# jkelleyrtp/ofdm

Hardware: AMD Instinct MI355X
Metric: complex IQ Msamples/s through RX demod (higher is better)
Workload: dtype f32; 1 GPU; cfg2: 64-subcarrier 64QAM guard-band frames, RX demod only (CP strip+FFT64+pilot phase+demap); frames_per_gpu=1000000, symbols_per_frame=16, samples_per_frame=1280, parallelism=frame-index split x1, no collective

## Files before the change

ofdm_amd/csrc/kernels_n64.hip:

```cpp
#include "device_common.hpp"
#include "kernels.hpp"
#include <type_traits>
#include <mutex>
#include <stdlib.h>

namespace ofdm {

typedef float f32x2 __attribute__((ext_vector_type(2)));
typedef __attribute__((address_space(3))) f32x2 *lds_cf_ptr;
typedef __attribute__((address_space(3))) unsigned *lds_u32_ptr;
template <int BPS, bool GUARD, bool HK, int BURST = 1>
__global__ __launch_bounds__(256, 4) void k_demod64(Fast64Params p) {
    constexpr int S = 80, CP = 16;
    constexpr int ND = GUARD ? 48 : 64;
    constexpr int REGION_DW = ND * BPS / 4;
    constexpr int SLAB = 8 * 72;

    __shared__ cf slab_all[4 * SLAB];
    __shared__ __align__(16) unsigned img_all[4 * BURST * REGION_DW];

    const int lane = threadIdx.x & 63;
    const int wave = __builtin_amdgcn_readfirstlane(threadIdx.x >> 6);
    const int s = lane >> 3, t = lane & 7;
    cf *buf = slab_all + wave * SLAB + s * 72;
    unsigned *img0 = img_all + wave * BURST * REGION_DW;

    cf w[7];
#pragma unroll
    for (int r = 1; r < 8; ++r) w[r - 1] = p.tw[r * t];
    cf g[8];
    if (HK) {
#pragma unroll
        for (int m = 0; m < 8; ++m) {
            cf h = p.hk[t + 8 * m];
            float ns = h.x * h.x + h.y * h.y;
            g[m] = make_float2(h.x / ns, -h.y / ns);
        }
    }
    unsigned wa[8], ra[8], fa[8], fs[8];
#pragma unroll
    for (int r = 0; r < 8; ++r) {
        wa[r] = pinned(lds_addr(buf + (swz(8 * t) ^ r)));
        ra[r] = pinned(lds_addr(buf + 8 * r + (t ^ r)));
        const int c = t + 8 * r;
        const int q = GUARD ? data_classes_below64(c) : c;
        const int bo = (s * ND + q) * BPS;
        const bool data = carrier_class64(c, GUARD) == 0;
        fa[r] = pinned(lds_addr(img0 + (bo >> 5)));
        fs[r] = pinned(data ? (unsigned)(bo & 31) : 0xFFFFFFFFu);
    }
    const int lane_off = s * S + t;

    auto group = [&](long long f, int kk, unsigned img_off) {
        const cf *src = p.in + f * p.frame_stride + (long long)(p.first_symbol + kk * 8) * S + CP + lane_off;
        cf v[8];
#pragma unroll
        for (int m = 0; m < 8; ++m) v[m] = src[8 * m];
        bfly8<false>(v);
        if (kProfile && p.debug == 3) {
            float acc = 0.f;
#pragma unroll
            for (int m = 0; m < 8; ++m) acc += v[m].x + v[m].y;
            if (acc == 12345.678f) p.out[0] = 1;
            return;
        }
#pragma unroll
        for (int r = 0; r < 8; ++r) *(lds_cf_ptr)(unsigned long)wa[r] = f32x2{v[r].x, v[r].y};
#pragma unroll
        for (int m = 0; m < 8; ++m) { const f32x2 q = *(lds_cf_ptr)(unsigned long)ra[m]; v[m] = make_float2(q.x, q.y); }
#pragma unroll
        for (int r = 1; r < 8; ++r) v[r] = cmul(v[r], w[r - 1]);
        bfly8<false>(v);
        if (HK) {
#pragma unroll
            for (int m = 0; m < 8; ++m) v[m] = cmul(v[m], g[m]);
        }
        cf rot = make_float2(1.f, 0.f);
        if (GUARD) {
            cf pv = make_float2(1.f, 0.f);
            pv = (t == 6) ? v[0] : pv;
            pv = (t == 1) ? v[3] : pv;
            pv = (t == 7) ? v[4] : pv;
            pv = (t == 2) ? v[7] : pv;
            const float turns = sum8_lanes(__ocml_atan2pi_f32(pv.y, pv.x)) * 0.125f;
            rot = make_float2(__builtin_amdgcn_cosf(turns), -__builtin_amdgcn_sinf(turns));
        }
        if (kProfile && p.debug == 2) {
            float acc = 0.f;
#pragma unroll
            for (int m = 0; m < 8; ++m) acc += v[m].x + v[m].y;
            if (acc == 12345.678f) p.out[0] = 1;
            return;
        }
        unsigned *img = reinterpret_cast<unsigned *>(reinterpret_cast<unsigned char *>(img0) + img_off);
        for (int i = lane; i < REGION_DW; i += 64) img[i] = 0u;
#pragma unroll
        for (int m = 0; m < 8; ++m) {
            const bool all_data = !GUARD || m == 1 || m == 2 || m == 5 || m == 6;
            if (all_data || fs[m] != 0xFFFFFFFFu) {
                const unsigned idx = GUARD ? demap_point_rot(v[m], rot, BPS) : demap_point(v[m], BPS);
                const lds_u32_ptr wd = (lds_u32_ptr)(unsigned long)(fa[m] + img_off);
                __hip_atomic_fetch_or(wd, idx << fs[m], __ATOMIC_RELAXED, __HIP_MEMORY_SCOPE_WORKGROUP);
                if (BPS > 1 && (32 % BPS) != 0) {
                    if (fs[m] + BPS > 32) __hip_atomic_fetch_or(wd + 1, idx >> (32 - fs[m]), __ATOMIC_RELAXED, __HIP_MEMORY_SCOPE_WORKGROUP);
                }
            }
        }
    };
    auto store_image = [&](unsigned *dst, int ndw) {
        if (kProfile && (p.debug == 1 || p.debug == 2 || p.debug == 3)) { if (img0[lane] == 0x12345678u) dst[0] = 1u; return; }
        if (kProfile && p.debug == 4) dst = reinterpret_cast<unsigned *>(p.out) + (blockIdx.x & 255) * 4 * BURST * REGION_DW + wave * BURST * REGION_DW;
        if (kProfile && p.debug == 5) { for (int i = lane; i < ndw; i += 64) __builtin_nontemporal_store(img0[i], dst + i); return; }
        if ((REGION_DW % 4) == 0 && p.wide_stores) {
            if (p.store_policy) {
                typedef unsigned v4u __attribute__((ext_vector_type(4)));
                for (int i = lane; i < ndw / 4; i += 64) {
                    const v4u val = reinterpret_cast<const v4u *>(img0)[i];
                    uint4 *a = reinterpret_cast<uint4 *>(dst) + i;
                    if (p.store_policy == 1) asm volatile("global_store_dwordx4 %0, %1, off nt" ::"v"(a), "v"(val) : "memory");
                    else if (p.store_policy == 2) asm volatile("global_store_dwordx4 %0, %1, off sc1" ::"v"(a), "v"(val) : "memory");
                    else asm volatile("global_store_dwordx4 %0, %1, off sc0 sc1" ::"v"(a), "v"(val) : "memory");
                }
                return;
            }
            for (int i = lane; i < ndw / 4; i += 64) reinterpret_cast<uint4 *>(dst)[i] = reinterpret_cast<const uint4 *>(img0)[i];
        } else for (int i = lane; i < ndw; i += 64) dst[i] = img0[i];
    };

    if (BURST > 1) {
        const long long n_bursts = p.n_groups / BURST;
        for (long long j = (long long)blockIdx.x * 4 + wave; j < n_bursts; j += p.stride_groups) {
            const long long g0 = j * BURST;
            long long f = g0 / p.groups_per_frame;
            int kk = (int)(g0 - f * p.groups_per_frame);
#pragma nounroll
            for (int b = 0; b < BURST; ++b) {
                group(f, kk, (unsigned)(b * REGION_DW * 4));
                if (++kk == p.groups_per_frame) { kk = 0; ++f; }
            }
            store_image(reinterpret_cast<unsigned *>(p.out + g0 * (long long)(REGION_DW * 4)), BURST * REGION_DW);
        }
        return;
    }

    long long f = p.f0 + (long long)blockIdx.x * p.blk_df + wave * p.wave_df;
    int kk = p.k0 + (int)((blockIdx.x * (long long)p.blk_dk + wave * p.wave_dk));
    f += kk / p.groups_per_frame;
    kk %= p.groups_per_frame;
    for (long long g_idx = (long long)blockIdx.x * 4 + wave; g_idx < p.n_groups; g_idx += p.stride_groups) {
        group(f, kk, 0u);
        store_image(reinterpret_cast<unsigned *>(p.out + f * p.out_stride + (long long)kk * 8 * (ND * BPS / 8)), REGION_DW);
        f += p.step_df;
        kk += p.step_dk;
        if (kk >= p.groups_per_frame) { kk -= p.groups_per_frame; f += 1; }
    }
}

struct RxFrame64Params {
    const float2 *in;
    long long n_frames, frame_stride, frame_len;
    const int32_t *offset;
    const double *f_delta;
    const int32_t *nsym;
    const float2 *tw, *inv_training;
    unsigned char *out;
    long long out_stride;
    float2 *hk;
    unsigned char *final_out;
    long long final_stride;
    int32_t *final_len;
    const int32_t *frame_list;
    const int32_t *frame_count;
    int32_t *cut_list;
    int32_t *cut_count;
};

__device__ __forceinline__ cf lane_xor_sum(cf v) {
    v.x += dpp_f<0x128>(v.x); v.y += dpp_f<0x128>(v.y);
    v.x += __shfl_xor(v.x, 16, 64); v.y += __shfl_xor(v.y, 16, 64);
    v.x += __shfl_xor(v.x, 32, 64); v.y += __shfl_xor(v.y, 32, 64);
    return v;
}

template <int BPS, bool GUARD, int MODE>
__global__ __launch_bounds__(256, (MODE == 0 && GUARD) ? 4 : 3) void k_rxframe64(RxFrame64Params p) {
    constexpr int S = 80, CP = 16;
    constexpr int ND = GUARD ? 48 : 64;
    constexpr int SYM_BYTES = ND * BPS / 8;
    constexpr int REGION_DW = ND * BPS / 4;
    constexpr int SLAB = 8 * 72;
    __shared__ cf slab_all[4 * SLAB];
    __shared__ cf ginv_all[4 * 64];
    __shared__ unsigned img_all[4 * REGION_DW];

    const int lane = threadIdx.x & 63;
    const int wave = __builtin_amdgcn_readfirstlane(threadIdx.x >> 6);
    const int s = lane >> 3, t = lane & 7;
    cf *buf = slab_all + wave * SLAB + s * 72;
    unsigned *img = img_all + wave * REGION_DW;

    __shared__ cf twl[64];
    __shared__ int bofftab[8 * 64];
    if (threadIdx.x < 64) twl[threadIdx.x] = p.tw[threadIdx.x];
    if (wave == 0) {
#pragma unroll
        for (int m = 0; m < 8; ++m) {
            const int c = t + 8 * m;
            const int q = GUARD ? data_classes_below64(c) : c;
            bofftab[m * 64 + lane] = (carrier_class64(c, GUARD) == 0) ? (s * ND + q) * BPS : -1;
        }
    }
    __shared__ int cutbuf[4][1 + 16];
    if (MODE == 0 && lane == 0) cutbuf[wave][0] = 0;
    __syncthreads();
    const int wr = swz(8 * t);
    auto cut_flush = [&]() {
        const int m = cutbuf[wave][0];
        if (m > 0) {
            const int base = atomicAdd(p.cut_count, m);
            for (int i = 0; i < m; ++i) p.cut_list[base + i] = cutbuf[wave][1 + i];
            cutbuf[wave][0] = 0;
        }
    };

    const long long n_items = p.frame_list ? (long long)*p.frame_count : p.n_frames;
    const long long istep = (long long)gridDim.x * 4;
    const int vzero = pinned(0);
    long long f_n = 0; int ns_v = 0, off_v = 0; double fd_v = 0.0;
    auto fetch_scalars = [&](long long item) {
        if (item < n_items) {
            f_n = p.frame_list ? (long long)p.frame_list[item] : item;
            const long long fi = f_n + vzero;
            ns_v = p.nsym[fi];
            off_v = p.offset ? p.offset[fi] : 0;
            fd_v = p.f_delta ? p.f_delta[fi] : 0.0;
        }
    };
    fetch_scalars((long long)blockIdx.x * 4 + wave);
    for (long long item = (long long)blockIdx.x * 4 + wave; item < n_items; item += istep) {
        const long long f = f_n;
        const int ns = __builtin_amdgcn_readfirstlane(ns_v);
        const long long off = __builtin_amdgcn_readfirstlane(off_v);
        const double turns = __hiloint2double(__builtin_amdgcn_readfirstlane(__double2hiint(fd_v)), __builtin_amdgcn_readfirstlane(__double2loint(fd_v))) * 0.15915494309189533577;
        fetch_scalars(item + istep);
        if (ns <= 0) { if (p.final_out && lane == 0) p.final_len[f] = 0; continue; }
        const cf st = cfo_phasor(turns, 8);
        int keep = 0;
        const cf *src = p.in + f * p.frame_stride + off;
        const long long avail = p.frame_len - off;

        auto frame_body = [&](auto cut_tag) {
        constexpr bool CUT = decltype(cut_tag)::value;
        const cf *safe = p.in + f * p.frame_stride + t;
        auto issue_group = [&](int k0, cf *v, unsigned &zmask) {
            const int count = ns - k0 < 8 ? ns - k0 : 8;
            const int n0 = (10 + k0 + s) * S + CP + t;
            const cf *base = s < count ? src + n0 : safe;
            zmask = 0u;
#pragma unroll
            for (int m = 0; m < 8; ++m) {
                const bool pad = CUT && s < count && (n0 + 8 * m) >= avail;
                v[m] = ld_cf(pad ? safe : base + 8 * m);
                if (CUT) zmask |= pad ? 1u << m : 0u;
            }
        };
        cf *ginv = ginv_all + wave * 64;
        cf v[8];
        unsigned zm = 0u;
        {
            cf tws[6];
            const int lq = pinned(lane);
#pragma unroll
            for (int q = 0; q < 6; ++q) {
                const int h = 32 >> q;
                const cf x = twl[(lq & (h - 1)) << q];
                tws[q] = (lane & h) ? x : make_float2(1.f, 0.f);
            }
            const int bin = bitrev6(lane);
            const cf invt = p.inv_training[bin];
            const int nb = 5 * S + CP + lane;
            cf xb[5];
#pragma unroll
            for (int b = 0; b < 5; ++b) xb[b] = ld_cf((!CUT || (nb + S * b) < avail) ? src + nb + S * b : safe);
            issue_group(0, v, zm);
#pragma unroll
            for (int b = 0; b < 5; ++b) if (CUT && (nb + S * b) >= avail) xb[b] = make_float2(0.f, 0.f);
            cf acc;
            if (p.f_delta) {
                const cf s80 = cfo_phasor(turns, S), q0 = cfo_phasor(turns, nb);
                acc = cadd(cmul(xb[4], s80), xb[3]);
                acc = cadd(cmul(acc, s80), xb[2]);
                acc = cadd(cmul(acc, s80), xb[1]);
                acc = cadd(cmul(acc, s80), xb[0]);
                acc = cmul(acc, q0);
            } else acc = cadd(cadd(cadd(xb[4], xb[3]), cadd(xb[2], xb[1])), xb[0]);
            acc = lane_fft64(acc, lane, tws);
            cf h = cmul(acc, invt);
            h = make_float2(h.x * 0.2f, h.y * 0.2f);
            if (p.hk) p.hk[f * 64 + bin] = h;
            const float rn = __builtin_amdgcn_rcpf(h.x * h.x + h.y * h.y);
            wave_fence();
            ginv[bin] = make_float2(h.x * rn, -h.y * rn);
            wave_fence();
        }
        for (int k0 = 0; k0 < ns; k0 += 8) {
            const int count = ns - k0 < 8 ? ns - k0 : 8;
            const int n0 = (10 + k0 + s) * S + CP + t;
            cf vn[8];
            unsigned zn = 0u;
            issue_group(k0 + 8 < ns ? k0 + 8 : k0, vn, zn);
            if (CUT && zm) {
#pragma unroll
                for (int m = 0; m < 8; ++m) if ((zm >> m) & 1u) v[m] = make_float2(0.f, 0.f);
            }
            if (p.f_delta) {
                cf ph = cfo_phasor(turns, n0);
#pragma unroll
                for (int m = 0; m < 8; ++m) { v[m] = cmul(v[m], ph); ph = cmul(ph, st); }
            }
            bfly8<false>(v);
#pragma unroll
            for (int r = 0; r < 8; ++r) buf[wr ^ r] = v[r];
#pragma unroll
            for (int m = 0; m < 8; ++m) v[m] = buf[8 * m + (t ^ m)];
#pragma unroll
            for (int r = 1; r < 8; ++r) v[r] = cmul(v[r], twl[r * t]);
            bfly8<false>(v);
#pragma unroll
            for (int m = 0; m < 8; ++m) v[m] = cmul(v[m], ginv[t + 8 * m]);
            cf rot = make_float2(1.f, 0.f);
            if (GUARD) {
                cf pv = make_float2(1.f, 0.f);
                pv = (t == 6) ? v[0] : pv;
                pv = (t == 1) ? v[3] : pv;
                pv = (t == 7) ? v[4] : pv;
                pv = (t == 2) ? v[7] : pv;
                const float trn = sum8_lanes(__ocml_atan2pi_f32(pv.y, pv.x)) * 0.125f;
                rot = make_float2(__builtin_amdgcn_cosf(trn), -__builtin_amdgcn_sinf(trn));
            }
            for (int i = lane; i < REGION_DW; i += 64) img[i] = 0u;
#pragma unroll
            for (int m = 0; m < 8; ++m) {
                const int bo = bofftab[m * 64 + lane];
                if (bo >= 0) {
                    const unsigned idx = GUARD ? demap_point_rot(v[m], rot, BPS) : demap_point(v[m], BPS);
                    or_field<BPS>(img, bo, idx);
                }
            }
#pragma unroll
            for (int m = 0; m < 8; ++m) v[m] = vn[m];
            zm = zn;
            const int ndw = (count * SYM_BYTES + 3) / 4;
            if (p.final_out) {
                wave_fence();
                if (k0 == 0) {
                    const unsigned long long lo = (unsigned long long)img[0] | ((unsigned long long)img[1] << 32);
                    const unsigned long long hi = (unsigned long long)img[2] | ((unsigned long long)img[3] << 32);
                    const int body = ns * SYM_BYTES - 16;
                    keep = OFDM_HEADER_KEEP(int, lo, hi, body);
                    if (lane == 0) p.final_len[f] = keep;
                }
                unsigned char *fo = p.final_out + f * p.final_stride;
                for (int i = lane; i < ndw; i += 64) {
                    const int ob = k0 * SYM_BYTES + 4 * i - 16;
                    if (ob < 0 || ob >= keep) continue;
                    if (ob + 4 <= keep) *reinterpret_cast<unsigned *>(fo + ob) = img[i];
                    else for (int j = 0; ob + j < keep; ++j) fo[ob + j] = (unsigned char)(img[i] >> (8 * j));
                }
            } else {
                unsigned *dst = reinterpret_cast<unsigned *>(p.out + f * p.out_stride + (long long)k0 * SYM_BYTES);
                for (int i = lane; i < ndw; i += 64) dst[i] = img[i];
            }
        }
        };
        const bool whole = (long long)(10 + ns) * S <= avail;
        if (MODE == 0) {
            if (whole) frame_body(std::false_type{});
            else if (lane == 0) {
                const int m = cutbuf[wave][0];
                cutbuf[wave][1 + m] = (int32_t)f;
                cutbuf[wave][0] = m + 1;
                if (m + 1 == 16) cut_flush();
            }
        } else if (MODE == 1) {
            if (!whole) frame_body(std::true_type{});
        } else {
            if (whole) frame_body(std::false_type{}); else frame_body(std::true_type{});
        }
    }
    if (MODE == 0 && lane == 0) cut_flush();
}

template <int BPS, bool GUARD> static hipError_t launch_rxframe(RxFrame64Params p, dim3 grid, hipStream_t st, bool split) {
    if (!split) { hipLaunchKernelGGL((k_rxframe64<BPS, GUARD, 2>), grid, dim3(256), 0, st, p); return hipGetLastError(); }
    hipError_t e = hipMemsetAsync(p.cut_count, 0, sizeof(int32_t), st);
    if (e != hipSuccess) return e;
    hipLaunchKernelGGL((k_rxframe64<BPS, GUARD, 0>), grid, dim3(256), 0, st, p);
    if ((e = hipGetLastError()) != hipSuccess) return e;
    p.frame_list = p.cut_list; p.frame_count = p.cut_count;
    hipLaunchKernelGGL((k_rxframe64<BPS, GUARD, 1>), grid, dim3(256), 0, st, p);
    return hipGetLastError();
}

hipError_t run_rxframe64(const SymParams &sp, float2 *hk_out, hipStream_t st, int num_cu, unsigned char *final_out,
                         long long final_stride, int32_t *final_len, const int32_t *frame_list, const int32_t *frame_count,
                         int32_t *cut_ws) {
    const int nd = sp.guard ? 48 : 64;
    if ((nd * sp.bps) % 16 != 0 || !sp.nsym_frame || sp.soft) return hipErrorNotSupported;
    const bool to_final = final_out && final_len && (reinterpret_cast<uintptr_t>(final_out) & 3) == 0 && (final_stride & 3) == 0;
    if (!to_final && ((reinterpret_cast<uintptr_t>(sp.out_bytes) & 3) || (sp.out_stride & 3))) return hipErrorNotSupported;
    if (sp.n_frames <= 0) return hipSuccess;
    RxFrame64Params p;
    p.in = sp.in; p.n_frames = sp.n_frames; p.frame_stride = sp.frame_stride; p.frame_len = sp.frame_len;
    p.offset = sp.offset; p.f_delta = sp.f_delta; p.nsym = sp.nsym_frame; p.tw = sp.tw; p.inv_training = sp.inv_training;
    p.out = sp.out_bytes; p.out_stride = sp.out_stride; p.hk = hk_out;
    p.final_out = nullptr; p.final_stride = 0; p.final_len = nullptr;
    if (to_final) { p.final_out = final_out; p.final_stride = final_stride; p.final_len = final_len; }
    else if (final_out) return hipErrorNotSupported;
    p.frame_list = frame_list; p.frame_count = frame_count;
    const bool roomy = sp.frame_len >= (long long)(10 + sp.syms_per_frame) * 80 + 64;
    const bool split = cut_ws != nullptr && frame_list == nullptr && roomy && !tuning_or_default(sp.tune).no_rxframe64_split;
    p.cut_count = split ? cut_ws : nullptr; p.cut_list = split ? cut_ws + 4 : nullptr;
    const dim3 grid((unsigned)persistent_grid((sp.n_frames + 3) / 4, frame_list ? 64 : (long long)num_cu * 8, tuning_or_default(sp.tune)));
    trace_add(sp.trace, frame_list ? "k_rxframe64<list>" : (p.final_out ? "k_rxframe64<finish>" : "k_rxframe64"));
    if (split) trace_add(sp.trace, "k_rxframe64<cut,list>");
    return with_bps(sp.bps, [&](auto B) { return with_bool(sp.guard != 0, [&](auto G) {
        return launch_rxframe<decltype(B)::value, decltype(G)::value>(p, grid, st, split); }); });
}

struct TxFrame64Params {
    const uint8_t *payload;
    long long payload_stride;
    const int32_t *payload_len;
    int payload_bytes;
    long long n_frames;
    int n_sym;
    const float2 *tw;
    const float2 *header;
    float header_max;
    float2 *out;
    long long out_stride;
    int debug;
};

template <int BPS, bool GUARD>
__global__ __launch_bounds__(256, 4) void k_txframe64(TxFrame64Params p) {
    constexpr int S = 80, CP = 16, HDR = 10 * S;
    constexpr int ND = GUARD ? 48 : 64;
    constexpr int SYM_BITS = ND * BPS;
    extern __shared__ __align__(16) unsigned char smem[];
    cf *hd = reinterpret_cast<cf *>(smem);
    cf *fb = hd + HDR;
    const int groups = (p.n_sym + 7) >> 3;
    unsigned *mxw = reinterpret_cast<unsigned *>(fb + (size_t)groups * 8 * S);
    unsigned *sbw_all = mxw + 4;
    const int sbw_dw = groups * 128 + 8;
    const int stream_dw = groups * 8 * (SYM_BITS / 8) / 4 + 1;

    const int tid = threadIdx.x, lane = tid & 63, nthr = blockDim.x, nwaves = nthr >> 6;
    const int wave = __builtin_amdgcn_readfirstlane(tid >> 6);
    const int s = lane >> 3, t = lane & 7;
    cf w[7];
#pragma unroll
    for (int r = 1; r < 8; ++r) { const cf x = p.tw[r * t]; w[r - 1] = make_float2(x.x, -x.y); }
    int qoff[8];
#pragma unroll
    for (int m = 0; m < 8; ++m) {
        const int c = t + 8 * m, cls = carrier_class64(c, GUARD);
        qoff[m] = cls == 0 ? (GUARD ? data_classes_below64(c) : c) * BPS : (cls == 2 ? -2 : -1);
    }
    const int wr = swz(8 * t);
    for (int i = tid; i < HDR; i += nthr) hd[i] = p.header[i];
    __shared__ float lvl[16];
    if (tid < 16) lvl[tid] = BPS > 1 && tid < (1 << (BPS >> 1)) ? axis_level((unsigned)tid, BPS >> 1) : 0.f;

    const bool aligned = ((reinterpret_cast<uintptr_t>(p.payload) | (uintptr_t)p.payload_stride) & 3) == 0;
    auto pay_dword = [&](const uint8_t *pay, long long len, int i) -> unsigned {
        const long long b0 = 4LL * i;
        if (b0 + 4 <= len && aligned) return reinterpret_cast<const unsigned *>(pay)[i];
        unsigned v = 0;
        for (int j = 0; j < 4; ++j) if (b0 + j < len) v |= (unsigned)pay[b0 + j] << (8 * j);
        return v;
    };
    const int vzero = pinned(0);
    const bool row0 = aligned && 4LL * tid + 4 <= p.payload_bytes, row1 = aligned && 4LL * (tid + nthr) + 4 <= p.payload_bytes;
    auto issue = [&](long long fr, unsigned &d0, unsigned &d1, int &ln) {
        const long long fc = fr < p.n_frames ? fr : p.n_frames - 1;
        const uint8_t *row = p.payload + fc * p.payload_stride;
        d0 = *reinterpret_cast<const unsigned *>(row0 ? row + 4 * tid : reinterpret_cast<const uint8_t *>(p.tw));
        d1 = *reinterpret_cast<const unsigned *>(row1 ? row + 4 * (tid + nthr) : reinterpret_cast<const uint8_t *>(p.tw));
        ln = p.payload_len ? p.payload_len[fc + vzero] : p.payload_bytes;
    };
    auto settle = [&](unsigned raw, bool whole, const uint8_t *pay, long long len, int i) -> unsigned {
        const long long keep = len - 4LL * i;
        if (whole) return keep >= 4 ? raw : (keep <= 0 ? 0u : raw & ((1u << (8 * (int)keep)) - 1u));
        return pay_dword(pay, len, i);
    };
    auto fill = [&](unsigned *sbw, long long fr, unsigned d0, unsigned d1, long long len) {
        const uint8_t *pay = p.payload + fr * p.payload_stride;
        if (tid < 4) sbw[tid] = tid < 2 ? (unsigned)((unsigned long long)len >> (32 * tid)) : 0u;
        if (tid + 4 < stream_dw) sbw[4 + tid] = settle(d0, row0, pay, len, tid);
        if (tid + nthr + 4 < stream_dw) sbw[4 + tid + nthr] = settle(d1, row1, pay, len, tid + nthr);
        for (int i = tid + 2 * nthr; i + 4 < stream_dw; i += nthr) sbw[4 + i] = pay_dword(pay, len, i);
    };
    long long f = blockIdx.x;
    unsigned pre0 = 0, pre1 = 0;
    int pre_len = 0;
    long long len = 0;
    int cur = 0;
    if (f < p.n_frames) {
        issue(f, pre0, pre1, pre_len);
        len = row_len(__builtin_amdgcn_readfirstlane(pre_len), p.payload_bytes);
        fill(sbw_all, f, pre0, pre1, len);
        issue(f + gridDim.x, pre0, pre1, pre_len);
    }
    if (tid < 2) mxw[tid] = 0u;
    for (; f < p.n_frames; f += gridDim.x, cur ^= 1) {
        lds_barrier();
        const long long t0 = kProfile && p.debug ? (long long)__builtin_amdgcn_s_memtime() : 0;
        const unsigned char *sb = reinterpret_cast<const unsigned char *>(sbw_all + cur * sbw_dw);
        long long t1 = 0;
        const int npoints = (int)(((16 + len) * 8 + BPS - 1) / BPS);
        float lmax = 0.f;
        for (int g = wave; g < groups; g += nwaves) {
            const int k = 8 * g + s;
            cf *buf = fb + k * S;
            cf v[8];
#pragma unroll
            for (int m = 0; m < 8; ++m) {
                cf z = make_float2(0.f, 0.f);
                if (qoff[m] == -2) z = make_float2(1.f, 0.f);
                else if (qoff[m] >= 0) {
                    const int bit = k * SYM_BITS + qoff[m];
                    if (bit < npoints * BPS && k < p.n_sym) {
                        const unsigned two = (unsigned)sb[bit >> 3] | ((unsigned)sb[(bit >> 3) + 1] << 8);
                        const unsigned idx = (two >> (bit & 7)) & ((1u << BPS) - 1u);
                        z = BPS == 1 ? map_point(idx, 1) : make_float2(lvl[idx & ((1u << (BPS >> 1)) - 1u)], lvl[idx >> (BPS >> 1)]);
                    }
                }
                v[m] = z;
            }
            bfly8<true>(v);
#pragma unroll
            for (int r = 0; r < 8; ++r) buf[wr ^ r] = v[r];
#pragma unroll
            for (int m = 0; m < 8; ++m) v[m] = buf[8 * m + (t ^ m)];
#pragma unroll
            for (int r = 1; r < 8; ++r) v[r] = cmul(v[r], w[r - 1]);
            bfly8<true>(v);
#pragma unroll
            for (int q = 0; q < 8; ++q) {
                const cf y = make_float2(v[q].x * (1.0f / 64), v[q].y * (1.0f / 64));
                v[q] = y;
                lmax = fmaxf(lmax, fmaxf(y.x, y.y));
            }
            wave_fence();
#pragma unroll
            for (int q = 0; q < 8; ++q) {
                buf[CP + t + 8 * q] = v[q];
                if (q >= 6) buf[t + 8 * q - 48] = v[q];
            }
        }
#pragma unroll
        for (int sh = 32; sh >= 1; sh >>= 1) lmax = fmaxf(lmax, __shfl_xor(lmax, sh, 64));
        if (lane == 0) atomicMax(&mxw[cur], __float_as_uint(lmax));
        if (kProfile && p.debug) t1 = (long long)__builtin_amdgcn_s_memtime();
        long long len_next = 0;
        if (f + gridDim.x < p.n_frames) {
            len_next = row_len(__builtin_amdgcn_readfirstlane(pre_len), p.payload_bytes);
            fill(sbw_all + (cur ^ 1) * sbw_dw, f + gridDim.x, pre0, pre1, len_next);
        }
        if (tid == 0) mxw[cur ^ 1] = 0u;
        issue(f + 2LL * gridDim.x, pre0, pre1, pre_len);
        lds_barrier();
        const long long t2 = kProfile && p.debug ? (long long)__builtin_amdgcn_s_memtime() : 0;
        const float inv = 1.0f / fmaxf(p.header_max, __uint_as_float(mxw[cur]));
        len = len_next;
        const int total2 = (HDR + p.n_sym * S) >> 1;
        float4 *dst = reinterpret_cast<float4 *>(p.out + f * p.out_stride);
        const float4 *src4 = reinterpret_cast<const float4 *>(hd);
        int i = tid;
        for (; i + 3 * nthr < total2; i += 4 * nthr) {
            const float4 a = src4[i], b = src4[i + nthr], c = src4[i + 2 * nthr], d = src4[i + 3 * nthr];
            dst[i] = make_float4(a.x * inv, a.y * inv, a.z * inv, a.w * inv);
            dst[i + nthr] = make_float4(b.x * inv, b.y * inv, b.z * inv, b.w * inv);
            dst[i + 2 * nthr] = make_float4(c.x * inv, c.y * inv, c.z * inv, c.w * inv);
            dst[i + 3 * nthr] = make_float4(d.x * inv, d.y * inv, d.z * inv, d.w * inv);
        }
        for (; i < total2; i += nthr) { const float4 a = src4[i]; dst[i] = make_float4(a.x * inv, a.y * inv, a.z * inv, a.w * inv); }
        if (kProfile && p.debug) {
            __syncthreads();
            if (tid == 0) {
                const long long t3 = (long long)__builtin_amdgcn_s_memtime();
                dst[0] = make_float4((float)(t1 - t0), (float)(t2 - t1), (float)(t3 - t2), 0.f);
            }
        }
    }
}

template <int BPS, bool GUARD> static hipError_t launch_txframe(const TxFrame64Params &p, dim3 grid, size_t lds, hipStream_t st) {
    const int groups = (p.n_sym + 7) / 8;
    const dim3 block(64u * (unsigned)(groups < 4 ? groups : 4));
    hipLaunchKernelGGL((k_txframe64<BPS, GUARD>), grid, block, lds, st, p);
    return hipGetLastError();
}
hipError_t run_txframe64(const SymParams &sp, const float2 *header, float header_max, hipStream_t st, int num_cu) {
    const int n_sym = sp.syms_per_frame;
    if (n_sym <= 0 || n_sym > 56 || (!sp.payload && sp.payload_bytes)) return hipErrorNotSupported;
    if ((reinterpret_cast<uintptr_t>(sp.out) & 15) || (sp.out_stride_s & 1)) return hipErrorNotSupported;
    if (sp.n_frames <= 0) return hipSuccess;
    TxFrame64Params p;
    p.payload = sp.payload; p.payload_stride = sp.payload_stride; p.payload_len = sp.payload_len; p.payload_bytes = sp.payload_bytes;
    p.n_frames = sp.n_frames; p.n_sym = n_sym; p.tw = sp.tw; p.header = header; p.header_max = header_max;
    p.out = sp.out; p.out_stride = sp.out_stride_s;
    const Tuning &tu = tuning_or_default(sp.tune);
    p.debug = kProfile ? tu.debug_tx : 0;
    const int groups = (n_sym + 7) / 8;
    const size_t lds = (size_t)(800 + groups * 8 * 80) * sizeof(float2) + 16 + 2 * ((size_t)groups * 8 * 64 + 32);
    long long per_cu = (long long)(160 * 1024) / (long long)lds;
    const int waves_per_cu = tu.tx_waves > 0 ? tu.tx_waves : 16;
    long long wave_cap = waves_per_cu / (groups < 4 ? groups : 4);
    if (wave_cap < 1) wave_cap = 1;
    if (per_cu > wave_cap) per_cu = wave_cap;
    const dim3 grid((unsigned)persistent_grid(sp.n_frames, (long long)num_cu * per_cu, tu));
    trace_add(sp.trace, "k_txframe64");
    return with_bps(sp.bps, [&](auto B) { return with_bool(sp.guard != 0, [&](auto G) {
        return launch_txframe<decltype(B)::value, decltype(G)::value>(p, grid, lds, st); }); });
}

template <typename K> static int resident_blocks(K kernel, int block) {
    struct Entry { const void *fn; int dev, n; };
    static Entry cache[64];
    static int used = 0;
    static std::mutex mtx;
    int dev = 0;
    if (hipGetDevice(&dev) != hipSuccess) dev = 0;
    const void *fn = reinterpret_cast<const void *>(kernel);
    std::lock_guard<std::mutex> lock(mtx);
    for (int i = 0; i < used; ++i) if (cache[i].fn == fn && cache[i].dev == dev) return cache[i].n;
    int n = 0;
    if (hipOccupancyMaxActiveBlocksPerMultiprocessor(&n, kernel, block, 0) != hipSuccess || n < 1) n = 4;
    n = n > 8 ? 8 : n;
    if (used < 64) cache[used++] = Entry{fn, dev, n};
    return n;
}
template <int BPS, bool GUARD, bool HK> static hipError_t launch_demod64(Fast64Params p, hipStream_t st, int num_cu, const Tuning &tu, Trace *trace) {
    p.debug = kProfile ? tu.debug_demod64 : 0;
    constexpr int region_bytes = (GUARD ? 48 : 64) * BPS;
    {
        p.store_policy = tu.demod64_store_policy;
        p.wide_stores = !tu.demod64_narrow_stores && region_bytes % 16 == 0 && (reinterpret_cast<uintptr_t>(p.out) & 15) == 0 && (p.out_stride & 15) == 0;
    }
    const bool burst = BPS == 6 && GUARD && !HK && tu.demod64_burst >= 4 && p.wide_stores && p.n_groups % 4 == 0 &&
                       p.out_stride == (long long)p.groups_per_frame * region_bytes && (reinterpret_cast<uintptr_t>(p.out) & 127) == 0;
    const int burst_cap = tu.demod64_burst;
    const int bl = !burst ? 1 : (burst_cap >= 16 && p.n_groups % 16 == 0) ? 16 : (burst_cap >= 8 && p.n_groups % 8 == 0) ? 8 : 4;
    auto kernel = !burst ? k_demod64<BPS, GUARD, HK, 1> : bl == 16 ? k_demod64<6, true, false, 16> : bl == 8 ? k_demod64<6, true, false, 8> : k_demod64<6, true, false, 4>;
    const long long units = burst ? p.n_groups / bl : p.n_groups;
    const int knob = tu.demod64_wg_per_cu;
    const int per_cu = knob > 0 ? knob : (resident_blocks(kernel, 256) >= 4 ? 8 : 2 * resident_blocks(kernel, 256));
    const int grid = (int)persistent_grid((units + 3) / 4, (long long)num_cu * per_cu, tu);
    trace_add(trace, !burst ? "k_demod64" : bl == 16 ? "k_demod64<burst16>" : bl == 8 ? "k_demod64<burst8>" : "k_demod64<burst4>");
    p.stride_groups = (long long)grid * 4;
    const int gpf = p.groups_per_frame;
    p.f0 = 0; p.k0 = 0;
    p.blk_df = 4 / gpf; p.blk_dk = 4 % gpf;
    p.wave_df = 0; p.wave_dk = 1;
    p.step_df = p.stride_groups / gpf; p.step_dk = (int)(p.stride_groups % gpf);
    hipLaunchKernelGGL(kernel, dim3(grid), dim3(256), 0, st, p);
    return hipGetLastError();
}

hipError_t run_demod64_fast(const SymParams &sp, hipStream_t st, int num_cu) {
    if (sp.offset || sp.f_delta || sp.nsym_frame || sp.soft) return hipErrorNotSupported;
    if (sp.syms_per_frame <= 0 || (sp.syms_per_frame & 7) != 0) return hipErrorNotSupported;
    if (sp.hk && sp.hk_stride != 0) return hipErrorNotSupported;
    if ((long long)(sp.first_symbol + sp.syms_per_frame) * 80 > sp.frame_len) return hipErrorNotSupported;
    if ((reinterpret_cast<uintptr_t>(sp.out_bytes) & 3) || (sp.out_stride & 3)) return hipErrorNotSupported;
    if (reinterpret_cast<uintptr_t>(sp.in) & 7) return hipErrorNotSupported;
    Fast64Params p;
    p.in = sp.in; p.frame_stride = sp.frame_stride; p.first_symbol = sp.first_symbol;
    p.hk = sp.hk; p.tw = sp.tw; p.out = sp.out_bytes; p.out_stride = sp.out_stride;
    p.groups_per_frame = sp.syms_per_frame / 8;
    p.n_groups = sp.n_frames * (long long)p.groups_per_frame;
    if (p.n_groups <= 0) return hipSuccess;
    const Tuning &tu = tuning_or_default(sp.tune);
    return with_bps(sp.bps, [&](auto B) { return with_bool(sp.guard != 0, [&](auto G) { return with_bool(p.hk != nullptr, [&](auto H) {
        return launch_demod64<decltype(B)::value, decltype(G)::value, decltype(H)::value>(p, st, num_cu, tu, sp.trace); }); }); });
}

}
```

Baseline: 828,900 Msamples/s.

## Double-buffer demap image and defer global stores to overlap with next group

Doubles the per-wave LDS bit-image buffer and defers each symbol group's global store until the next group's loads have been issued, so store traffic overlaps demod compute. The output write loop becomes fixed-trip with byte-range masks, and the header keep length is computed from wave-uniform reads. Adds pinned() on the FFT inputs and nounroll on the group loop to limit register pressure and code size. The extra LDS could lower occupancy, and the deferred flush state adds bookkeeping, including a flush after the item loop.

```diff
diff --git a/ofdm_amd/csrc/kernels_n64.hip b/ofdm_amd/csrc/kernels_n64.hip
--- a/ofdm_amd/csrc/kernels_n64.hip
+++ b/ofdm_amd/csrc/kernels_n64.hip
@@ -191,13 +191,14 @@
     constexpr int SLAB = 8 * 72;
     __shared__ cf slab_all[4 * SLAB];
     __shared__ cf ginv_all[4 * 64];
-    __shared__ unsigned img_all[4 * REGION_DW];
+    constexpr int NST = (REGION_DW + 63) / 64;
+    __shared__ unsigned img_all[4 * 2 * REGION_DW];
 
     const int lane = threadIdx.x & 63;
     const int wave = __builtin_amdgcn_readfirstlane(threadIdx.x >> 6);
     const int s = lane >> 3, t = lane & 7;
     cf *buf = slab_all + wave * SLAB + s * 72;
-    unsigned *img = img_all + wave * REGION_DW;
+    unsigned *img2 = img_all + wave * 2 * REGION_DW;
 
     __shared__ cf twl[64];
     __shared__ int bofftab[8 * 64];
@@ -236,6 +237,39 @@
             fd_v = p.f_delta ? p.f_delta[fi] : 0.0;
         }
     };
+    int cur = 0;
+    long long pend_f = 0;
+    int pend_k0 = 0, pend_keep = 0;
+    int pend_hi = 0;
+    auto flush_pending = [&]() {
+        if (pend_hi <= 0) return;
+        const unsigned *im = img2 + (cur ^ 1) * REGION_DW;
+        unsigned char *base;
+        int lo = 0;
+        if (p.final_out) {
+            base = p.final_out + pend_f * p.final_stride + ((long long)pend_k0 * SYM_BYTES - 16);
+            if (pend_k0 == 0) {
+                lo = 16;
+                if (lane == 0) p.final_len[pend_f] = pend_keep;
+            }
+        } else base = p.out + pend_f * p.out_stride + (long long)pend_k0 * SYM_BYTES;
+#pragma unroll
+        for (int j = 0; j < NST; ++j) {
+            const int b = 4 * (lane + 64 * j);
+            if (b >= lo && b + 4 <= pend_hi) *reinterpret_cast<unsigned *>(base + b) = im[lane + 64 * j];
+        }
+        if (p.final_out && (pend_hi & 3)) {
+            const int i = pend_hi >> 2, r = pend_hi & 3;
+            if (lane == (i & 63)) {
+                const unsigned w = im[i];
+                base[4 * i] = (unsigned char)w;
+                if (r > 1) base[4 * i + 1] = (unsigned char)(w >> 8);
+                if (r > 2) base[4 * i + 2] = (unsigned char)(w >> 16);
+            }
+        }
+        pend_hi = 0;
+    };
+
     fetch_scalars((long long)blockIdx.x * 4 + wave);
     for (long long item = (long long)blockIdx.x * 4 + wave; item < n_items; item += istep) {
         const long long f = f_n;
@@ -303,12 +337,17 @@
             ginv[bin] = make_float2(h.x * rn, -h.y * rn);
             wave_fence();
         }
+#pragma unroll
+        for (int m = 0; m < 8; ++m) { v[m].x = pinned(v[m].x); v[m].y = pinned(v[m].y); }
+#pragma nounroll
         for (int k0 = 0; k0 < ns; k0 += 8) {
             const int count = ns - k0 < 8 ? ns - k0 : 8;
             const int n0 = (10 + k0 + s) * S + CP + t;
             cf vn[8];
             unsigned zn = 0u;
             issue_group(k0 + 8 < ns ? k0 + 8 : k0, vn, zn);
+            flush_pending();
+            unsigned *img = img2 + cur * REGION_DW;
             if (CUT && zm) {
 #pragma unroll
                 for (int m = 0; m < 8; ++m) if ((zm >> m) & 1u) v[m] = make_float2(0.f, 0.f);
@@ -347,30 +386,23 @@
                     or_field<BPS>(img, bo, idx);
                 }
             }
+            int hi_b = 4 * ((count * SYM_BYTES + 3) / 4);
+            wave_fence();
+            if (p.final_out) {
+                if (k0 == 0) {
+                    const unsigned long long lo = (unsigned long long)(unsigned)uniform((int)img[0]) | ((unsigned long long)(unsigned)uniform((int)img[1]) << 32);
+                    const unsigned long long hi = (unsigned long long)(unsigned)uniform((int)img[2]) | ((unsigned long long)(unsigned)uniform((int)img[3]) << 32);
+                    const int body = ns * SYM_BYTES - 16;
+                    keep = OFDM_HEADER_KEEP(int, lo, hi, body);
+                }
+                const int end = keep + 16 - k0 * SYM_BYTES;
+                hi_b = end < hi_b ? (end > 0 ? end : 0) : hi_b;
+            }
+            pend_f = f; pend_k0 = k0; pend_keep = keep; pend_hi = hi_b;
+            cur ^= 1;
 #pragma unroll
             for (int m = 0; m < 8; ++m) v[m] = vn[m];
             zm = zn;
-            const int ndw = (count * SYM_BYTES + 3) / 4;
-            if (p.final_out) {
-                wave_fence();
-                if (k0 == 0) {
-                    const unsigned long long lo = (unsigned long long)img[0] | ((unsigned long long)img[1] << 32);
-                    const unsigned long long hi = (unsigned long long)img[2] | ((unsigned long long)img[3] << 32);
-                    const int body = ns * SYM_BYTES - 16;
-                    keep = OFDM_HEADER_KEEP(int, lo, hi, body);
-                    if (lane == 0) p.final_len[f] = keep;
-                }
-                unsigned char *fo = p.final_out + f * p.final_stride;
-                for (int i = lane; i < ndw; i += 64) {
-                    const int ob = k0 * SYM_BYTES + 4 * i - 16;
-                    if (ob < 0 || ob >= keep) continue;
-                    if (ob + 4 <= keep) *reinterpret_cast<unsigned *>(fo + ob) = img[i];
-                    else for (int j = 0; ob + j < keep; ++j) fo[ob + j] = (unsigned char)(img[i] >> (8 * j));
-                }
-            } else {
-                unsigned *dst = reinterpret_cast<unsigned *>(p.out + f * p.out_stride + (long long)k0 * SYM_BYTES);
-                for (int i = lane; i < ndw; i += 64) dst[i] = img[i];
-            }
         }
         };
         const bool whole = (long long)(10 + ns) * S <= avail;
@@ -388,6 +420,7 @@
             if (whole) frame_body(std::false_type{}); else frame_body(std::true_type{});
         }
     }
+    flush_pending();
     if (MODE == 0 && lane == 0) cut_flush();
 }
 
```

Measured after the change: 815,400 Msamples/s. -1.6%, worse.
